# TomClabault/RayTracerCPP

Hardware: NVIDIA B200
Metric: Mrays/s (primary+shadow) (higher is better)
Workload: dtype f32

## Files before the change

### raytracercpp_b200/csrc/kernels.cuh

```cuda
#pragma once

#include <cuda_runtime.h>
#include "rt_device.h"

namespace rtb {

constexpr int kPatch = 8;
constexpr int kPrimaryThreads = 128;
constexpr int kQueueThreads = 128;
constexpr int kPrimaryFetch = 1;
constexpr int kStepsPerCheck = 4;
constexpr unsigned kParkCtas = 296;
constexpr unsigned kFusedGenerations = 12;
constexpr int kItemPasses = 6;
#ifndef RTB_SHADE_MINB
#define RTB_SHADE_MINB 7
#endif

constexpr int kSubQueues = 32;
struct alignas(128) SubQueue {
    unsigned int n;
    unsigned int next;
    unsigned int pad[30];
};
// ... 52 lines not shown
        f += __shfl_xor_sync(0xffffffffu, f, o);
    }
    if ((threadIdx.x & 31u) == 0) {
        if (v) atomicAdd(vol, v);
        if (t) atomicAdd(tri, t);
        if (f) atomicAdd(fetch, f);
    }
}

struct WorkView {
    const uint32_t* tiles;
    uint32_t tile_begin, tile_end;
    int32_t tiles_x;
    int32_t tile_px;
    int32_t patches_per_side;
    int32_t cull_x0, cull_y0, cull_x1, cull_y1;
};

struct QueueView {
    int32_t* slot_tri;
    float* slot_t;
    float* slot_u;
    float* slot_v;
    uint32_t* hit_slot;
    uint32_t* hit_sorted;
    uint32_t sort_mode, sort_slots;
    float* g_z;
    V3* g_n;
    uint32_t* split_base;
    uint32_t* split_active;
    uint32_t* split_occ;
// ... 9 lines not shown
    uint32_t capacity;
};

RT_DEV bool slot_pixel(const WorkView& wk, const FrameView& fr, uint32_t slot, int& px, int& py)
{
    const uint32_t pps = (uint32_t)wk.patches_per_side;
    const uint32_t per_tile = pps * pps * (uint32_t)(kPatch * kPatch);
    const uint32_t tile = wk.tiles[wk.tile_begin + slot / per_tile];
    const uint32_t in_tile = slot % per_tile;
    const uint32_t patch = in_tile / (uint32_t)(kPatch * kPatch), in_patch = in_tile % (uint32_t)(kPatch * kPatch);
    const int lx = (int)(patch % pps) * kPatch + (int)(in_patch & 7u);
    const int ly = (int)(patch / pps) * kPatch + (int)(in_patch >> 3);
    px = (int)(tile % (uint32_t)wk.tiles_x) * wk.tile_px + lx;
    py = (int)(tile / (uint32_t)wk.tiles_x) * wk.tile_px + ly;
    return lx < wk.tile_px && ly < wk.tile_px && px < fr.rw && py < fr.rh;
}

struct Tuning {
    int32_t primary_refill;
    int32_t shade_refill;
    int32_t tri_batch;
    int32_t packets;
    int32_t packet_rounds;
    int32_t item_rounds;
    int32_t primary_rounds;
    int32_t fused;
    int32_t packet_min, item_min, primary_min;
    int32_t item_passes;
    int32_t cull;
};
// ... 455 lines not shown
    uint32_t traced = 0;
    uint32_t nxt = 0;
    if (lane == 0) nxt = atomicAdd(&cnt->next_patch, 32u * kPrimaryFetch);
    for (;;) {
        const uint32_t first = __shfl_sync(0xffffffffu, nxt, 0);
        if (first >= total) break;
        if (lane == 0) nxt = atomicAdd(&cnt->next_patch, 32u * kPrimaryFetch);
#pragma unroll 1
        for (uint32_t b = 0; b < (uint32_t)kPrimaryFetch; b++) {
            const uint32_t base = first + 32u * b;
            if (base >= total) break;
            const uint32_t slot = base + lane;
            int px = 0, py = 0;
            const bool active = slot < total && slot_pixel(wk, fr, slot, px, py);
            V3 o = v3(0, 0, 0), d = v3(0, 0, 1);
            const bool inside = active && px >= wk.cull_x0 && px <= wk.cull_x1 && py >= wk.cull_y0 && py <= wk.cull_y1;
            if (__ballot_sync(0xffffffffu, inside) == 0u) {
                if (slot < total) {
                    q.slot_tri[slot] = -1;
                    if (active) {
                        if (miss_needs_ray(fr)) primary_ray(fr, px, py, o, d);
                        super[(size_t)py * fr.rw + px] = quantise_argb(shade_miss(sc, fr, d));
                    }
                }
                continue;
            }
            if (active) primary_ray(fr, px, py, o, d);
            traced += (uint32_t)__popc(__ballot_sync(0xffffffffu, active));
            HitRec best;
            bool occ, live = active;
            unsigned rounds = 0;
// ... 1173 lines not shown
            backoff = min(backoff * 2u, 4000u);
            continue;
        }
        const uint32_t base = __shfl_sync(0xffffffffu, nxt, 0);
        if (base >= total) {
            more = false;
            if (lane == 0 && my_packets && tune.primary_rounds > 0) { __threadfence(); atomicAdd(&cnt->ft[0].packets_done, my_packets); }
            continue;
        }
        if (lane == 0) nxt = atomicAdd(&cnt->next_patch, 32u);
        rem = (total - base) / per_round;
        const uint32_t slot = base + lane;
        int px = 0, py = 0;
        const bool active = slot_pixel(wk, fr, slot, px, py);
        V3 o = v3(0, 0, 0), d = v3(0, 0, 1);
        const bool inside = active && px >= wk.cull_x0 && px <= wk.cull_x1 && py >= wk.cull_y0 && py <= wk.cull_y1;
        bool deferred = false;
        if (__ballot_sync(0xffffffffu, inside) == 0u) {
            q.slot_tri[slot] = -1;
            if (active) {
                if (miss_needs_ray(fr)) primary_ray(fr, px, py, o, d);
                super[(size_t)py * fr.rw + px] = quantise_argb(shade_miss(sc, fr, d));
            }
        } else {
            if (active) primary_ray(fr, px, py, o, d);
            traced += (uint32_t)__popc(__ballot_sync(0xffffffffu, active));
            HitRec best;
            bool occ, live = active;
            unsigned rounds = 0;
            const unsigned long long t0 = COUNT ? global_ns() : 0ull;
            const bool finished = packet_trace<false, COUNT>(sc, K, top, live, o, d, INFINITY, o, 0.0f, best, occ, tc, overflow,
// ... 183 lines not shown
```

### raytracercpp_b200/csrc/octree_device.cuh

```cuda
#pragma once

#include "scene_layout.h"

namespace rtb {
namespace devbuild {

constexpr int kExtraLevels = 0;
constexpr int kMaxKeyLevels = 21;
constexpr int kSortRounds = 64;
constexpr int kSortUnit = 32 * kSortRounds;
constexpr int kScanItems = 4;
constexpr int kScanBlock = 1024 * kScanItems;

struct Params {
    int32_t max_depth, leaf_max, leaf_split, total_depth;
    float s3;
};

struct Stats {
    unsigned long long interior, nonempty_children;
    unsigned int max_depth, max_leaf;
    unsigned int root_lo[3], root_hi[3];
    unsigned int top_n;
};
// ... 585 lines not shown

__global__ void __launch_bounds__(256)
k_wb_records(const float4* recs, const uint32_t* src, Cells C, uint32_t n_nodes, float4* wrecs)
{
    const uint32_t node = blockIdx.x * blockDim.x + threadIdx.x;
    if (node >= n_nodes) return;
    const float4* s = recs + 4 * (size_t)src[node];
    float4* q = wrecs + 4 * (size_t)C.rec[node];
    float4 q3 = s[3];
    const uint32_t kids = C.info[node] & 15u;
    if (kids) { q3.z = __uint_as_float(C.block[node]); q3.w = __uint_as_float(kids); }
    q[0] = s[0]; q[1] = s[1]; q[2] = s[2]; q[3] = q3;
}

__global__ void __launch_bounds__(256)
k_ob_transform(float* xyz, size_t n_vertices, M4 t)
{
    for (size_t i = (size_t)blockIdx.x * blockDim.x + threadIdx.x; i < n_vertices; i += (size_t)gridDim.x * blockDim.x) {
        const V3 p = xform_point(t, v3(xyz[3 * i], xyz[3 * i + 1], xyz[3 * i + 2]));
        xyz[3 * i] = p.x; xyz[3 * i + 1] = p.y; xyz[3 * i + 2] = p.z;
    }
}

}
}
```

### raytracercpp_b200/csrc/rtb200.cu

```cuda
#include "../../include/rtb200.h"

#include <cuda_runtime.h>
#include <omp.h>
#include <sched.h>

#include <algorithm>
#include <atomic>
#include <chrono>
#include <cmath>
#include <cstdarg>
#include <cstdio>
#include <cstdlib>
#include <cstring>
#include <map>
#include <string>
#include <tuple>
#include <vector>

#include "kernels.cuh"
#include "scene_layout.h"
#include "octree_device.cuh"
#include "light_cull.cuh"
#include "ssao.cuh"
#include "raster.cuh"
#include "host_common.h"

using namespace rtb;

namespace {

constexpr uint64_t kChunkPixels = 1ull << 28;
constexpr int kMaxChunks = 256;

thread_local std::string g_create_error;
std::atomic<unsigned long long> g_alloc_generation{0};

double now_ms()
{
    return std::chrono::duration<double, std::milli>(std::chrono::steady_clock::now().time_since_epoch()).count();
}

template <typename T>
struct DevBuf {
    T* p = nullptr;
    size_t n = 0;
    cudaError_t ensure(size_t count)
    {
// ... 24 lines not shown

struct TimedLaunch {
    int stage;
    cudaEvent_t a, b;
    const char* label;
};

struct TileList {
    uint32_t* d = nullptr;
    uint32_t count = 0;
    int tiles_x = 0;
    std::vector<uint32_t> host;
    uint32_t* d_split = nullptr;
    std::vector<uint32_t> split_host;
    uint32_t n_traced = 0;
    int32_t split_rect[4] = {0, 0, -1, -1};
    int32_t split_tile_px = 0;
    bool split_valid = false;
    float last_hit_fraction = -1.0f;
};
typedef std::tuple<int, int, int, int, int> TileKey;

}

constexpr int kLanes = 2;
constexpr int kMaxLanes = 6;

struct QueueSet {
    DevBuf<uint32_t> hit_slot, refl_idx, split_base, split_active, split_occ, item_ready, split_pending;
    DevBuf<uint32_t> hit_sorted, sort_keys, sort_bins;
    DevBuf<unsigned long long> split_best, refl_cnt;
// ... 16 lines not shown
    bool count = false, shadow = false;
    bool raster = false;
    cudaEvent_t ev_begin = nullptr, ev_end = nullptr;
    uint64_t primary_rays = 0;
    bool has_key = false;
    int key[5] = {0, 0, 0, 0, 0};
    uint64_t traced_slots = 0;
};

struct DeviceBuild {
    DevBuf<float> xyz9, uv6, centroid, c_nr, c_fr;
    DevBuf<int32_t> mat;
    DevBuf<unsigned long long> keys[2];
    DevBuf<uint32_t> idx[2], hist, sums, counts, c_begin, c_end, c_first, c_info, c_size, c_rec, c_block;
    DevBuf<uint32_t> w_src, w_members;
    DevBuf<devbuild::Stats> stats;
    bool tris_on_device = false;
    std::vector<M4> host_pending;
    void release()
    {
        xyz9.release(); uv6.release(); centroid.release(); c_nr.release(); c_fr.release(); mat.release(); keys[0].release(); keys[1].release();
        idx[0].release(); idx[1].release(); hist.release(); sums.release(); counts.release(); c_begin.release(); c_end.release(); c_first.release();
        c_info.release(); c_size.release(); c_rec.release(); c_block.release(); w_src.release(); w_members.release(); stats.release();
    }
};

struct RtContext {
    int device = 0;
    int sm_count = 0;
    cudaStream_t stream = nullptr;
    cudaStream_t own_stream = nullptr;
    std::string error;

    std::vector<float> xyz9, uv6;
    std::vector<int32_t> mat;
    bool has_uv = false, has_mat = false;
    int32_t max_mat_index = -1, min_mat_index = 0;

// ... 54 lines not shown
    DevBuf<RasterUnit> d_runits;
    DevBuf<unsigned int> d_rcount;
    DevBuf<float4> d_rfrag;
    size_t raster_smem_set = 0;
    bool opt_graph = true;
    bool opt_fan_lanes = true;
    bool capturing = false;
    struct FrameGraph { std::string key; cudaGraphExec_t exec; uint32_t launches; };
    std::vector<FrameGraph> graphs;
    std::vector<std::string> seen_keys;
    size_t raster_units0 = (size_t)1 << 18;
    M4 proj{};
    float proj_fov = 45.0f, proj_aspect = 1.0f;
    bool proj_set = false;
    float root_lo[3] = {0, 0, 0}, root_hi[3] = {0, 0, 0};

    bool opt_light_cull = true;
    DevBuf<uint32_t> d_tri_occ, d_blk_occ, d_rec_parent;
    struct LightMaskInputs { V3 light; float span; uint32_t all_set; uint64_t tree; } mask_in{}, mask_next{};
    uint32_t mask_words = 0, mask_recs = 0;
    bool mask_valid = false;
    uint64_t mask_generation = 0;

    DevBuf<float> b_a, b_b, b_t, b_u, b_v;
    DevBuf<int32_t> b_id;
    DevBuf<uint8_t> b_occ;
};

namespace {

// ... 212 lines not shown
        for (int r = c + 1; r < 4; r++) if (std::fabs(m[r][c]) > std::fabs(m[piv][c])) piv = r;
        if (std::fabs(m[piv][c]) < 1e-300) return false;
        if (piv != c) for (int j = 0; j < 8; j++) std::swap(m[piv][j], m[c][j]);
        const double d = 1.0 / m[c][c];
        for (int j = 0; j < 8; j++) m[c][j] *= d;
        for (int r = 0; r < 4; r++) {
            if (r == c) continue;
            const double f = m[r][c];
            if (f != 0.0) for (int j = 0; j < 8; j++) m[r][j] -= f * m[c][j];
        }
    }
    for (int i = 0; i < 4; i++) for (int j = 0; j < 4; j++) out[4 * i + j] = m[i][4 + j];
    return true;
}

void screen_cull_rect(const RtContext* ctx, const FrameView& fr, WorkView& wk)
{
    wk.cull_x0 = 0; wk.cull_y0 = 0; wk.cull_x1 = fr.rw - 1; wk.cull_y1 = fr.rh - 1;
    if (!ctx->opt_screen_cull) return;
    if (ctx->n_tris == 0 || !(ctx->root_lo[0] <= ctx->root_hi[0])) { wk.cull_x0 = 1; wk.cull_x1 = 0; return; }
    double c2w[16], pinv[16], w2c[16], proj[16];
    for (int i = 0; i < 16; i++) { c2w[i] = (&ctx->cam_to_world.m[0][0])[i]; pinv[i] = (&ctx->proj_inv.m[0][0])[i]; }
    if (!invert4(c2w, w2c) || !invert4(pinv, proj)) return;
    const double w0 = c2w[15];
    if (!(std::fabs(w0) > 1e-12)) return;
    const double centre[3] = {c2w[3] / w0, c2w[7] / w0, c2w[11] / w0};
    const double pos[3] = {ctx->cam_pos.x, ctx->cam_pos.y, ctx->cam_pos.z};
    double scale = 1.0;
    for (int k = 0; k < 3; k++) scale = std::max(scale, std::fabs(centre[k]));
    for (int k = 0; k < 3; k++) if (std::fabs(centre[k] - pos[k]) > 1e-5 * scale) return;
    double xmin = 1e300, xmax = -1e300, ymin = 1e300, ymax = -1e300;
    for (int corner = 0; corner < 8; corner++) {
        const double p[4] = {corner & 1 ? ctx->root_hi[0] : ctx->root_lo[0], corner & 2 ? ctx->root_hi[1] : ctx->root_lo[1],
                             corner & 4 ? ctx->root_hi[2] : ctx->root_lo[2], 1.0};
        double v[4], c[4];
        for (int i = 0; i < 4; i++) v[i] = w2c[4 * i] * p[0] + w2c[4 * i + 1] * p[1] + w2c[4 * i + 2] * p[2] + w2c[4 * i + 3] * p[3];
        if (!(std::fabs(v[3]) > 1e-12)) return;
        for (int i = 0; i < 3; i++) v[i] /= v[3];
        v[3] = 1.0;
        for (int i = 0; i < 4; i++) c[i] = proj[4 * i] * v[0] + proj[4 * i + 1] * v[1] + proj[4 * i + 2] * v[2] + proj[4 * i + 3] * v[3];
        if (!(c[3] > 1e-3 * (1.0 + std::fabs(v[2])))) return;
        const double nx = c[0] / c[3], ny = c[1] / c[3];
        if (!std::isfinite(nx) || !std::isfinite(ny)) return;
        xmin = std::min(xmin, nx); xmax = std::max(xmax, nx); ymin = std::min(ymin, ny); ymax = std::max(ymax, ny);
    }
    for (int k = 0; k < 5; k++) {
        const double nx = k == 4 ? 0.0 : (k & 1 ? 1.0 : -1.0), ny = k == 4 ? 0.0 : (k & 2 ? 1.0 : -1.0);
        double v[4];
        for (int i = 0; i < 4; i++) v[i] = pinv[4 * i] * nx + pinv[4 * i + 1] * ny - pinv[4 * i + 2] + pinv[4 * i + 3];
        if (!(std::fabs(v[3]) > 1e-12)) return;
        for (int i = 0; i < 3; i++) v[i] /= v[3];
        for (const double along : {1.0, 7.5}) {
            const double q[4] = {v[0] * along, v[1] * along, v[2] * along, 1.0};
            double c[4];
            for (int i = 0; i < 4; i++) c[i] = proj[4 * i] * q[0] + proj[4 * i + 1] * q[1] + proj[4 * i + 2] * q[2] + proj[4 * i + 3] * q[3];
            if (!(c[3] > 0.0) || !(std::fabs(c[0] / c[3] - nx) < 1e-4) || !(std::fabs(c[1] / c[3] - ny) < 1e-4)) return;
        }
    }
    const double px0 = (xmin + 1.0) * 0.5 * fr.rw, px1 = (xmax + 1.0) * 0.5 * fr.rw;
    const double py0 = (ymin + 1.0) * 0.5 * fr.rh, py1 = (ymax + 1.0) * 0.5 * fr.rh;
    const double lim = 1e9;
    wk.cull_x0 = (int32_t)std::max(-lim, std::floor(px0) - 2.0); wk.cull_x1 = (int32_t)std::min(lim, std::ceil(px1) + 2.0);
    wk.cull_y0 = (int32_t)std::max(-lim, std::floor(py0) - 2.0); wk.cull_y1 = (int32_t)std::min(lim, std::ceil(py1) + 2.0);
}

int get_tile_list(RtContext* ctx, const RtSettings* s, int tile_size, int tile_mod, int tile_rem, TileList** out)
{
    const TileKey key(s->image_width, s->image_height, tile_size, tile_mod, tile_rem);
    auto it = ctx->tile_lists.find(key);
    if (it == ctx->tile_lists.end()) {
        if (ctx->tile_lists.size() > 64) {
            RT_CUDA(ctx, cudaStreamSynchronize(ctx->stream));
            for (auto& kv : ctx->tile_lists) { cudaFree(kv.second.d); cudaFree(kv.second.d_split); }
            ctx->tile_lists.clear();
        }
        TileList tl;
        if (tile_rem >= 0) tl.host = owned_tiles(s, tile_size, tile_mod, tile_rem, &tl.tiles_x);
        else {
// ... 72 lines not shown
}

int scan_counts(RtContext* ctx, uint32_t* data, size_t count, uint32_t* total)
{
    using namespace devbuild;
    DeviceBuild& D = ctx->db;
    const cudaStream_t st = ctx->stream;
    const uint32_t blocks = (uint32_t)((count + kScanBlock - 1) / kScanBlock);
    RT_CUDA(ctx, D.sums.ensure(std::max<uint32_t>(blocks, 1)));
    k_scan_sums<<<blocks, 1024, 0, st>>>(data, count, D.sums.p);
    k_scan_top<<<1, 1024, 0, st>>>(D.sums.p, blocks, total);
    k_scan_apply<<<blocks, 1024, 0, st>>>(data, count, D.sums.p);
    return RT_OK;
}

int build_wide_tree(RtContext* ctx, uint64_t n_records)
{
    using namespace devbuild;
    DeviceBuild& D = ctx->db;
    const cudaStream_t st = ctx->stream;
    const size_t cap = (size_t)n_records;
    RT_CUDA(ctx, D.w_src.ensure(cap)); RT_CUDA(ctx, D.c_first.ensure(cap)); RT_CUDA(ctx, D.c_info.ensure(cap)); RT_CUDA(ctx, D.c_size.ensure(cap));
    RT_CUDA(ctx, D.c_rec.ensure(cap)); RT_CUDA(ctx, D.c_block.ensure(cap)); RT_CUDA(ctx, D.stats.ensure(1));
    Cells C;
    memset(&C, 0, sizeof(C));
    C.first_child = D.c_first.p; C.info = D.c_info.p; C.size = D.c_size.p; C.rec = D.c_rec.p; C.block = D.c_block.p;
    {
        const uint32_t zero = 0u, root_block = 2u;
        RT_CUDA(ctx, cudaMemcpyAsync(D.w_src.p, &zero, 4, cudaMemcpyHostToDevice, st));
        RT_CUDA(ctx, cudaMemcpyAsync(C.rec, &zero, 4, cudaMemcpyHostToDevice, st));
// ... 6 lines not shown
    for (;;) {
        const uint32_t lf = level_first.back(), lc = level_count.back();
        RT_CUDA(ctx, D.counts.ensure(lc));
        RT_CUDA(ctx, D.w_members.ensure(8 * (size_t)lc));
        k_wb_collapse<<<(lc + 255) / 256, 256, 0, st>>>(recs, D.w_src.p, lf, lc, C.info, D.counts.p, D.w_members.p);
        if (int r = scan_counts(ctx, D.counts.p, lc, d_total)) return r;
        uint32_t total = 0;
        RT_CUDA(ctx, cudaMemcpyAsync(&total, d_total, 4, cudaMemcpyDeviceToHost, st));
        RT_CUDA(ctx, cudaStreamSynchronize(st));
        if (total == 0) break;
        if ((size_t)lf + lc + total > cap) return fail(ctx, RT_ERR_STATE, "wide tree: more nodes than child records");
        k_wb_children<<<(lc + 255) / 256, 256, 0, st>>>(C, D.w_src.p, lf, lc, D.counts.p, D.w_members.p, lf + lc);
        level_first.push_back(lf + lc); level_count.push_back(total);
    }
    const uint32_t n_nodes = level_first.back() + level_count.back();
    for (int l = (int)level_first.size() - 1; l >= 0; l--)
        k_wb_size<<<(level_count[l] + 255) / 256, 256, 0, st>>>(C, level_first[l], level_count[l]);
    uint32_t root_size = 0;
    RT_CUDA(ctx, cudaMemcpyAsync(&root_size, C.size, 4, cudaMemcpyDeviceToHost, st));
    RT_CUDA(ctx, cudaStreamSynchronize(st));
    const uint64_t n_wide = 2ull + root_size;
    ctx->n_wrecs = n_wide;
    RT_CUDA(ctx, ctx->d_wrecs.ensure(4 * n_wide));
    RT_CUDA(ctx, cudaMemsetAsync(ctx->d_wrecs.p, 0, 4 * n_wide * sizeof(float4), st));
    Params P;
    memset(&P, 0, sizeof(P));
    for (size_t l = 0; l < level_first.size(); l++)
        k_ob_place<<<(level_count[l] + 255) / 256, 256, 0, st>>>(C, level_first[l], level_count[l], P);
    k_wb_records<<<(n_nodes + 255) / 256, 256, 0, st>>>(recs, D.w_src.p, C, n_nodes, (float4*)ctx->d_wrecs.p);
    k_ob_top_table<<<1, 32, 0, st>>>((float4*)ctx->d_wrecs.p, (float4*)ctx->d_top.p, D.stats.p);
// ... 138 lines not shown
    const bool packets_wide = P.leaf_split > 0;
    if (!packets_wide) k_ob_top_table<<<1, 32, 0, st>>>((float4*)ctx->d_recs.p, (float4*)ctx->d_top.p, D.stats.p);
    Stats hs;
    F4 root_rec[2];
    RT_CUDA(ctx, cudaMemcpyAsync(&hs, D.stats.p, sizeof(hs), cudaMemcpyDeviceToHost, st));
    RT_CUDA(ctx, cudaMemcpyAsync(root_rec, ctx->d_recs.p, sizeof(root_rec), cudaMemcpyDeviceToHost, st));
    RT_CUDA(ctx, cudaStreamSynchronize(st));
    RT_CUDA(ctx, cudaGetLastError());
    ctx->top_n = (int)hs.top_n;
    if (packets_wide) if (int r = build_wide_tree(ctx, n_records)) return r;
    const double t2 = now_ms();

    ctx->n_tris = n32;
    ctx->root_lo[0] = root_rec[0].x; ctx->root_lo[1] = root_rec[0].z; ctx->root_lo[2] = root_rec[1].x;
    ctx->root_hi[0] = root_rec[0].y; ctx->root_hi[1] = root_rec[0].w; ctx->root_hi[2] = root_rec[1].y;
    RtBvhInfo& bi = ctx->info;
    bi.triangles = n;
    bi.interior = hs.interior;
    bi.nodes = 1 + 8 * hs.interior;
    bi.leaves = bi.nodes - bi.interior;
    bi.empty_leaves = 8 * hs.interior - hs.nonempty_children;
    bi.max_depth_reached = hs.max_depth; bi.max_leaf_size = hs.max_leaf;
    bi.child_records = n_records;
    bi.device_bytes = (4 * n_records + 3 * n + 2 * n) * sizeof(F4) + n * sizeof(int32_t);
    bi.build_ms = t2 - t1;
    bi.upload_ms = t1 - t0;
    ctx->bvh_valid = true;
    if (getenv("RTB200_TRACE"))
        fprintf(stderr, "[rtb200] device octree: %u cells on %zu levels, %llu records, upload %.1f ms, build %.1f ms\n", n_cells, level_first.size(),
                (unsigned long long)n_records, t1 - t0, t2 - t1);
// ... 191 lines not shown
    ctx->bvh_valid = false;
    ctx->db.tris_on_device = false;
    ctx->db.host_pending.clear();
    return RT_OK;
}

int rt_build_bvh(RtContext* ctx, int max_depth, int leaf_max_obj_count)
{
    if (!ctx) return RT_ERR_INVALID;
    if (int r = bind(ctx)) return r;
    if (max_depth < 0 || max_depth > RT_MAX_TREE_DEPTH) return fail(ctx, RT_ERR_INVALID, "max_depth %d outside [0,%d]", max_depth, RT_MAX_TREE_DEPTH);
    if (leaf_max_obj_count < 0) return fail(ctx, RT_ERR_INVALID, "leaf_max_obj_count %d", leaf_max_obj_count);
    const size_t n = ctx->xyz9.size() / 9;
    ctx->bvh_valid = false;
    ctx->wide_tree = false;
    ctx->tree_serial++;
    if (ctx->opt_device_build && n > 0) return build_bvh_device(ctx, max_depth, leaf_max_obj_count);
    apply_pending_host_transforms(ctx);
    double t0 = now_ms();
    FlatScene flat;
    build_flat_scene(ctx->xyz9.data(), ctx->has_uv ? ctx->uv6.data() : nullptr, ctx->has_mat ? ctx->mat.data() : nullptr, n,
                     max_depth, leaf_max_obj_count, ctx->opt_leaf_split, flat);
    double t1 = now_ms();
    if (flat.n_records >= (1ull << 28)) return fail(ctx, RT_ERR_INVALID, "scene needs %llu child records (limit 2^28)", (unsigned long long)flat.n_records);
    RT_CUDA(ctx, cudaStreamSynchronize(ctx->stream));
    RT_CUDA(ctx, ctx->d_recs.ensure(flat.recs.size()));
    RT_CUDA(ctx, ctx->d_tris.ensure(flat.tris.size()));
    RT_CUDA(ctx, ctx->d_shade.ensure(flat.shade.size()));
    RT_CUDA(ctx, ctx->d_orig.ensure(flat.orig.size()));
    RT_CUDA(ctx, ctx->d_leaf_of.ensure(flat.orig.size()));
// ... 9 lines not shown
        RT_CUDA(ctx, cudaMemcpyAsync(ctx->d_shade.p, flat.shade.data(), flat.shade.size() * sizeof(F4), cudaMemcpyHostToDevice, ctx->stream));
        RT_CUDA(ctx, cudaMemcpyAsync(ctx->d_orig.p, flat.orig.data(), flat.orig.size() * sizeof(int32_t), cudaMemcpyHostToDevice, ctx->stream));
        RT_CUDA(ctx, cudaMemcpyAsync(ctx->d_leaf_of.p, leaf_of.data(), leaf_of.size() * sizeof(int32_t), cudaMemcpyHostToDevice, ctx->stream));
    }
    RT_CUDA(ctx, cudaStreamSynchronize(ctx->stream));
    double t2 = now_ms();
    if (n && ctx->opt_leaf_split > 0)
        if (int r = build_wide_tree(ctx, flat.n_records)) return r;
    const double wide_ms = now_ms() - t2;
    ctx->n_tris = (uint32_t)n;
    {
        const F4 *q0 = &flat.recs[0], *q1 = &flat.recs[1];
        ctx->root_lo[0] = q0->x; ctx->root_lo[1] = q0->z; ctx->root_lo[2] = q1->x;
        ctx->root_hi[0] = q0->y; ctx->root_hi[1] = q0->w; ctx->root_hi[2] = q1->y;
    }
    RtBvhInfo& bi = ctx->info;
    bi.triangles = n;
    bi.nodes = flat.nodes; bi.leaves = flat.leaves; bi.empty_leaves = flat.empty_leaves; bi.interior = flat.interior;
    bi.max_depth_reached = flat.max_depth_reached; bi.max_leaf_size = flat.max_leaf_size;
    bi.child_records = flat.n_records;
    bi.device_bytes = (flat.recs.size() + flat.tris.size() + flat.shade.size()) * sizeof(F4) + flat.orig.size() * sizeof(int32_t);
    bi.build_ms = t1 - t0 + wide_ms;
    bi.upload_ms = t2 - t1;
    ctx->bvh_valid = true;
    return RT_OK;
}

int rt_bvh_info(const RtContext* ctx, RtBvhInfo* out)
{
    if (!ctx || !out) return RT_ERR_INVALID;
// ... 121 lines not shown
    if (!(aspect > 0.0f) || !(zfar > znear)) return fail(ctx, RT_ERR_INVALID, "projection: aspect %g, znear %g, zfar %g", aspect, znear, zfar);
    ctx->proj = perspective_matrix(fov, aspect, znear, zfar);
    ctx->proj_fov = fov;
    ctx->proj_aspect = aspect;
    ctx->proj_set = true;
    return RT_OK;
}

int rt_set_light(RtContext* ctx, const float position[3])
{
    if (!ctx || !position) return RT_ERR_INVALID;
    ctx->light = v3(position[0], position[1], position[2]);
    return RT_OK;
}

int rt_tile_count(const RtSettings* s, int tile_size, int tile_mod, int tile_rem)
{
    if (!s || tile_size <= 0 || tile_mod <= 0 || tile_rem < 0 || tile_rem >= tile_mod) return RT_ERR_INVALID;
    return (int)owned_tiles(s, tile_size, tile_mod, tile_rem, nullptr).size();
}

int rt_render_device_begin(RtContext* ctx, const RtSettings* s, uint32_t* d_argb_out, int tile_size, int tile_mod, int tile_rem)
{
    if (!ctx) return RT_ERR_INVALID;
    if (ctx->pending.active) return fail(ctx, RT_ERR_STATE, "rt_render_device_begin: the previous frame has not been ended (rt_render_device_end)");
    if (int r = bind(ctx)) return r;
    if (int r = validate_settings(ctx, s)) return r;
    if (int r = validate_scene_for_render(ctx, s)) return r;
    if (int r = check_tile_args(ctx, tile_size, tile_mod, tile_rem)) return r;
    if (!d_argb_out) return fail(ctx, RT_ERR_INVALID, "d_argb_out is NULL");
// ... 10 lines not shown
    const FrameView fr = frame_view(ctx, s);
    const SceneView sc = scene_view(ctx);
    const SceneView scp = packet_view(ctx);
    const bool resolve = fr.factor > 1;
    const bool reflect = ctx->any_reflective && s->shading_method == RT_SHADING;
    if (reflect) if (int r = ensure_stack(ctx, s)) return r;

    TileList* tl = nullptr;
    if (int r = get_tile_list(ctx, s, tile_size, tile_mod, tile_rem, &tl)) return r;
    const std::vector<uint32_t>& owned = tl->host;
    const int tiles_x = tl->tiles_x;
    WorkView wk = {};
    wk.tiles_x = tiles_x;
    wk.tile_px = tile_size * fr.factor;
    wk.patches_per_side = (wk.tile_px + kPatch - 1) / kPatch;
    screen_cull_rect(ctx, fr, wk);
    const bool has_shapes = !ctx->shapes.empty();
    if (has_shapes) { wk.cull_x0 = 0; wk.cull_y0 = 0; wk.cull_x1 = fr.rw - 1; wk.cull_y1 = fr.rh - 1; }
    const bool classify = ctx->opt_screen_cull && ctx->tune.packets && tl->count > 0 && !has_shapes && !raster;
    if (classify) {
        const int32_t rect[4] = {wk.cull_x0, wk.cull_y0, wk.cull_x1, wk.cull_y1};
        if (!tl->split_valid || memcmp(rect, tl->split_rect, sizeof(rect)) != 0 || tl->split_tile_px != wk.tile_px) {
            std::vector<uint32_t> in, out;
            for (uint32_t tile : owned) {
                const int x0 = (int)(tile % (uint32_t)tiles_x) * wk.tile_px, y0 = (int)(tile / (uint32_t)tiles_x) * wk.tile_px;
                const bool hit = !(x0 + wk.tile_px - 1 < rect[0] || x0 > rect[2] || y0 + wk.tile_px - 1 < rect[1] || y0 > rect[3]);
                (hit ? in : out).push_back(tile);
            }
            tl->n_traced = (uint32_t)in.size();
            tl->split_host = in;
            tl->split_host.insert(tl->split_host.end(), out.begin(), out.end());
            if (!tl->d_split) RT_CUDA(ctx, cudaMalloc((void**)&tl->d_split, tl->count * sizeof(uint32_t)));
            RT_CUDA(ctx, cudaStreamSynchronize(ctx->stream));
            RT_CUDA(ctx, cudaMemcpy(tl->d_split, tl->split_host.data(), tl->count * sizeof(uint32_t), cudaMemcpyHostToDevice));
            memcpy(tl->split_rect, rect, sizeof(rect));
            tl->split_tile_px = wk.tile_px;
            tl->split_valid = true;
        }
    }
    const uint32_t n_traced = raster ? 0u : (classify ? tl->n_traced : tl->count);
    const std::vector<uint32_t> tiles(classify ? tl->split_host.begin() : owned.begin(), (classify ? tl->split_host.begin() : owned.begin()) + n_traced);
    const uint64_t px_per_tile = (uint64_t)wk.patches_per_side * wk.patches_per_side * kPatch * kPatch;
    uint32_t tiles_per_chunk = (uint32_t)std::max<uint64_t>(1, ctx->opt_chunk_pixels / px_per_tile);
    if ((tiles.size() + tiles_per_chunk - 1) / tiles_per_chunk > (size_t)kMaxChunks)
        tiles_per_chunk = (uint32_t)((tiles.size() + kMaxChunks - 1) / kMaxChunks);
    const int n_lanes = (ctx->opt_lanes > 1 && tune_packets_hint(ctx)) ? (int)std::min<size_t>((size_t)ctx->opt_lanes, std::max<size_t>(tiles.size(), 1)) : 1;
    if (n_lanes > 1 && tiles.size() <= (size_t)tiles_per_chunk * (n_lanes - 1)) tiles_per_chunk = (uint32_t)((tiles.size() + n_lanes - 1) / n_lanes);
    std::vector<uint32_t> bounds;
    for (size_t b = 0; b < tiles.size(); b += tiles_per_chunk) bounds.push_back((uint32_t)b);
    bounds.push_back((uint32_t)tiles.size());
// ... 101 lines not shown
    bool replay = false, capture = false;
    size_t graph_at = 0;
    std::string key;
    if (graph_ok) {
        auto put = [&](const void* ptr, size_t n) { key.append((const char*)ptr, n); };
        auto put64 = [&](unsigned long long v) { put(&v, sizeof(v)); };
        put(&sc, sizeof(sc)); put(&scp, sizeof(scp)); put(&fr, sizeof(fr)); put(&wk, sizeof(wk)); put(qv, sizeof(QueueView) * (size_t)n_lanes); put(&tune, sizeof(tune));
        put(&light_map, sizeof(light_map));
        if (!bounds.empty()) put(bounds.data(), bounds.size() * sizeof(uint32_t));
        put64((unsigned long long)tile_size); put64((unsigned long long)tile_mod); put64((unsigned long long)tile_rem); put64((unsigned long long)n_lanes);
        put64(n_chunks); put64(classify); put64(n_traced); put64(tl->count); put64((unsigned long long)(uintptr_t)tl->d); put64((unsigned long long)(uintptr_t)tl->d_split);
        put64(sort_hits); put64((unsigned long long)ctx->opt_shadow_sort); put64(tail); put64(psplit); put64(reflect); put64(ssao); put64(resolve); put64(count); put64(has_shapes);
        put64(ctx->opt_top_table); put64((unsigned long long)(uintptr_t)d_argb_out); put64((unsigned long long)(uintptr_t)super);
        put64((unsigned long long)(uintptr_t)ctx->d_counters.p); put64((unsigned long long)(uintptr_t)pd.host_cnt); put64(g_alloc_generation.load());
        put64((unsigned long long)(uintptr_t)main_stream); put64((unsigned long long)split_cap); put64((unsigned long long)item_cap); put64(px_per_tile);
        put64((unsigned long long)ctx->stack_limit_set); put64(ctx->opt_fan_lanes); put64(ctx->mask_generation);
        if (ssao) { put(&ctx->proj, sizeof(ctx->proj)); put(&ctx->proj_fov, sizeof(float)); put(&ctx->proj_aspect, sizeof(float)); }
        for (size_t i = 0; i < ctx->graphs.size() && !replay; i++)
            if (ctx->graphs[i].key == key) { replay = true; graph_at = i; }
        if (!replay) {
            for (const std::string& k : ctx->seen_keys) capture |= (k == key);
            if (!capture) {
                if (ctx->seen_keys.size() >= 4) ctx->seen_keys.erase(ctx->seen_keys.begin());
                ctx->seen_keys.push_back(key);
            }
        }
    }
    cudaEvent_t ev_begin = next_event(ctx), ev_end = next_event(ctx);
    RT_CUDA(ctx, cudaEventRecord(ev_begin, st));
    if (rebuild_masks) if (int r = build_light_masks(ctx, st)) return r;
    auto enqueue = [&]() -> int {
// ... 637 lines not shown
```

Before: 22820.

## Replace screen-space cull rectangle with per-block coverage bitmap from upper tree boxes

Replaces the single screen rectangle (the projected root box) with a bitmap of 8x4 pixel blocks. The bitmap is built on the host by projecting up to 4096 boxes from an upper level of the wide tree, each padded by a conservative error margin. Primary rays in uncovered blocks, and whole tiles with no covered blocks, skip traversal and are shaded as misses. The cost is extra host work and a device-to-host box copy at build time, a bitmap upload when the camera changes, and one bitmap load per ray.

```diff
diff --git a/raytracercpp_b200/csrc/kernels.cuh b/raytracercpp_b200/csrc/kernels.cuh
--- a/raytracercpp_b200/csrc/kernels.cuh
+++ b/raytracercpp_b200/csrc/kernels.cuh
@@ -90,7 +90,8 @@
     int32_t tiles_x;
     int32_t tile_px;
     int32_t patches_per_side;
-    int32_t cull_x0, cull_y0, cull_x1, cull_y1;
+    const uint32_t* cover;
+    int32_t cover_words;
 };
 
 struct QueueView {
@@ -130,6 +131,13 @@
     px = (int)(tile % (uint32_t)wk.tiles_x) * wk.tile_px + lx;
     py = (int)(tile / (uint32_t)wk.tiles_x) * wk.tile_px + ly;
     return lx < wk.tile_px && ly < wk.tile_px && px < fr.rw && py < fr.rh;
+}
+
+RT_DEV bool covered(const WorkView& wk, int px, int py)
+{
+    if (wk.cover == nullptr) return true;
+    const uint32_t w = __ldg(wk.cover + ((uint32_t)py >> 2) * (uint32_t)wk.cover_words + ((uint32_t)px >> 8));
+    return ((w >> (((uint32_t)px >> 3) & 31u)) & 1u) != 0u;
 }
 
 struct Tuning {
@@ -615,7 +623,7 @@
             int px = 0, py = 0;
             const bool active = slot < total && slot_pixel(wk, fr, slot, px, py);
             V3 o = v3(0, 0, 0), d = v3(0, 0, 1);
-            const bool inside = active && px >= wk.cull_x0 && px <= wk.cull_x1 && py >= wk.cull_y0 && py <= wk.cull_y1;
+            const bool inside = active && covered(wk, px, py);
             if (__ballot_sync(0xffffffffu, inside) == 0u) {
                 if (slot < total) {
                     q.slot_tri[slot] = -1;
@@ -1819,7 +1827,7 @@
         int px = 0, py = 0;
         const bool active = slot_pixel(wk, fr, slot, px, py);
         V3 o = v3(0, 0, 0), d = v3(0, 0, 1);
-        const bool inside = active && px >= wk.cull_x0 && px <= wk.cull_x1 && py >= wk.cull_y0 && py <= wk.cull_y1;
+        const bool inside = active && covered(wk, px, py);
         bool deferred = false;
         if (__ballot_sync(0xffffffffu, inside) == 0u) {
             q.slot_tri[slot] = -1;
diff --git a/raytracercpp_b200/csrc/octree_device.cuh b/raytracercpp_b200/csrc/octree_device.cuh
--- a/raytracercpp_b200/csrc/octree_device.cuh
+++ b/raytracercpp_b200/csrc/octree_device.cuh
@@ -623,6 +623,18 @@
 }
 
 __global__ void __launch_bounds__(256)
+k_wb_boxes(const float4* recs, const uint32_t* src, const uint32_t* info, uint32_t n, uint32_t first_kept, float* boxes)
+{
+    const uint32_t node = blockIdx.x * blockDim.x + threadIdx.x;
+    if (node >= n) return;
+    const float4 q0 = recs[4 * (size_t)src[node]], q1 = recs[4 * (size_t)src[node] + 1];
+    const bool keep = node >= first_kept || (info[node] & 15u) == 0u;
+    float* b = boxes + 6 * (size_t)node;
+    b[0] = keep ? q0.x : INFINITY; b[1] = keep ? q0.z : INFINITY; b[2] = keep ? q1.x : INFINITY;
+    b[3] = keep ? q0.y : -INFINITY; b[4] = keep ? q0.w : -INFINITY; b[5] = keep ? q1.y : -INFINITY;
+}
+
+__global__ void __launch_bounds__(256)
 k_ob_transform(float* xyz, size_t n_vertices, M4 t)
 {
     for (size_t i = (size_t)blockIdx.x * blockDim.x + threadIdx.x; i < n_vertices; i += (size_t)gridDim.x * blockDim.x) {
diff --git a/raytracercpp_b200/csrc/rtb200.cu b/raytracercpp_b200/csrc/rtb200.cu
--- a/raytracercpp_b200/csrc/rtb200.cu
+++ b/raytracercpp_b200/csrc/rtb200.cu
@@ -31,6 +31,7 @@
 
 constexpr uint64_t kChunkPixels = 1ull << 28;
 constexpr int kMaxChunks = 256;
+constexpr uint32_t kCoverBoxes = 4096;
 
 thread_local std::string g_create_error;
 std::atomic<unsigned long long> g_alloc_generation{0};
@@ -85,7 +86,7 @@
     uint32_t* d_split = nullptr;
     std::vector<uint32_t> split_host;
     uint32_t n_traced = 0;
-    int32_t split_rect[4] = {0, 0, -1, -1};
+    uint64_t split_cover = 0;
     int32_t split_tile_px = 0;
     bool split_valid = false;
     float last_hit_fraction = -1.0f;
@@ -132,6 +133,7 @@
     DevBuf<unsigned long long> keys[2];
     DevBuf<uint32_t> idx[2], hist, sums, counts, c_begin, c_end, c_first, c_info, c_size, c_rec, c_block;
     DevBuf<uint32_t> w_src, w_members;
+    DevBuf<float> w_boxes;
     DevBuf<devbuild::Stats> stats;
     bool tris_on_device = false;
     std::vector<M4> host_pending;
@@ -139,7 +141,7 @@
     {
         xyz9.release(); uv6.release(); centroid.release(); c_nr.release(); c_fr.release(); mat.release(); keys[0].release(); keys[1].release();
         idx[0].release(); idx[1].release(); hist.release(); sums.release(); counts.release(); c_begin.release(); c_end.release(); c_first.release();
-        c_info.release(); c_size.release(); c_rec.release(); c_block.release(); w_src.release(); w_members.release(); stats.release();
+        c_info.release(); c_size.release(); c_rec.release(); c_block.release(); w_src.release(); w_members.release(); w_boxes.release(); stats.release();
     }
 };
 
@@ -224,6 +226,14 @@
     float proj_fov = 45.0f, proj_aspect = 1.0f;
     bool proj_set = false;
     float root_lo[3] = {0, 0, 0}, root_hi[3] = {0, 0, 0};
+    std::vector<float> cover_boxes;
+    struct CoverInputs { M4 proj_inv, cam_to_world; V3 cam_pos; int32_t rw, rh; uint64_t tree; } cover_in{};
+    bool cover_valid = false;
+    bool cover_bound = false;
+    int32_t cover_words = 0;
+    std::vector<uint32_t> h_cover;
+    DevBuf<uint32_t> d_cover;
+    uint64_t cover_generation = 0;
 
     bool opt_light_cull = true;
     DevBuf<uint32_t> d_tri_occ, d_blk_occ, d_rec_parent;
@@ -466,54 +476,188 @@
     return true;
 }
 
-void screen_cull_rect(const RtContext* ctx, const FrameView& fr, WorkView& wk)
-{
-    wk.cull_x0 = 0; wk.cull_y0 = 0; wk.cull_x1 = fr.rw - 1; wk.cull_y1 = fr.rh - 1;
-    if (!ctx->opt_screen_cull) return;
-    if (ctx->n_tris == 0 || !(ctx->root_lo[0] <= ctx->root_hi[0])) { wk.cull_x0 = 1; wk.cull_x1 = 0; return; }
+bool screen_coverage(const M4& cam_to_world, const M4& proj_inv, V3 cam_pos, int rw, int rh, const float* boxes, size_t n_boxes,
+                     double margin_scale, std::vector<uint32_t>& bits, int32_t& words_per_row)
+{
+    const int bw = (rw + 7) / 8, bh = (rh + 3) / 4;
+    words_per_row = (bw + 31) / 32;
+    bits.assign((size_t)words_per_row * (size_t)bh, 0u);
+    auto set_blocks = [&](int bx0, int by0, int bx1, int by1) {
+        for (int by = by0; by <= by1; by++) {
+            uint32_t* row = bits.data() + (size_t)by * words_per_row;
+            for (int w = bx0 >> 5; w <= bx1 >> 5; w++) {
+                const int lo = std::max(bx0 - 32 * w, 0), hi = std::min(bx1 - 32 * w, 31);
+                row[w] |= (hi == 31 ? 0xffffffffu : ((1u << (hi + 1)) - 1u)) & ~((1u << lo) - 1u);
+            }
+        }
+    };
+    if (n_boxes == 0) return true;
     double c2w[16], pinv[16], w2c[16], proj[16];
-    for (int i = 0; i < 16; i++) { c2w[i] = (&ctx->cam_to_world.m[0][0])[i]; pinv[i] = (&ctx->proj_inv.m[0][0])[i]; }
-    if (!invert4(c2w, w2c) || !invert4(pinv, proj)) return;
+    for (int i = 0; i < 16; i++) { c2w[i] = (&cam_to_world.m[0][0])[i]; pinv[i] = (&proj_inv.m[0][0])[i]; }
+    if (!invert4(c2w, w2c) || !invert4(pinv, proj)) return false;
     const double w0 = c2w[15];
-    if (!(std::fabs(w0) > 1e-12)) return;
+    if (!(std::fabs(w0) > 1e-12)) return false;
     const double centre[3] = {c2w[3] / w0, c2w[7] / w0, c2w[11] / w0};
-    const double pos[3] = {ctx->cam_pos.x, ctx->cam_pos.y, ctx->cam_pos.z};
-    double scale = 1.0;
+    const double pos[3] = {cam_pos.x, cam_pos.y, cam_pos.z};
+    double scale = 1.0, dc = 0.0;
     for (int k = 0; k < 3; k++) scale = std::max(scale, std::fabs(centre[k]));
-    for (int k = 0; k < 3; k++) if (std::fabs(centre[k] - pos[k]) > 1e-5 * scale) return;
-    double xmin = 1e300, xmax = -1e300, ymin = 1e300, ymax = -1e300;
-    for (int corner = 0; corner < 8; corner++) {
-        const double p[4] = {corner & 1 ? ctx->root_hi[0] : ctx->root_lo[0], corner & 2 ? ctx->root_hi[1] : ctx->root_lo[1],
-                             corner & 4 ? ctx->root_hi[2] : ctx->root_lo[2], 1.0};
-        double v[4], c[4];
-        for (int i = 0; i < 4; i++) v[i] = w2c[4 * i] * p[0] + w2c[4 * i + 1] * p[1] + w2c[4 * i + 2] * p[2] + w2c[4 * i + 3] * p[3];
-        if (!(std::fabs(v[3]) > 1e-12)) return;
-        for (int i = 0; i < 3; i++) v[i] /= v[3];
-        v[3] = 1.0;
-        for (int i = 0; i < 4; i++) c[i] = proj[4 * i] * v[0] + proj[4 * i + 1] * v[1] + proj[4 * i + 2] * v[2] + proj[4 * i + 3] * v[3];
-        if (!(c[3] > 1e-3 * (1.0 + std::fabs(v[2])))) return;
-        const double nx = c[0] / c[3], ny = c[1] / c[3];
-        if (!std::isfinite(nx) || !std::isfinite(ny)) return;
-        xmin = std::min(xmin, nx); xmax = std::max(xmax, nx); ymin = std::min(ymin, ny); ymax = std::max(ymax, ny);
-    }
+    for (int k = 0; k < 3; k++) {
+        if (!(std::fabs(centre[k] - pos[k]) <= 1e-5 * scale)) return false;
+        dc += (centre[k] - pos[k]) * (centre[k] - pos[k]);
+    }
+    dc = std::sqrt(dc);
     for (int k = 0; k < 5; k++) {
         const double nx = k == 4 ? 0.0 : (k & 1 ? 1.0 : -1.0), ny = k == 4 ? 0.0 : (k & 2 ? 1.0 : -1.0);
         double v[4];
         for (int i = 0; i < 4; i++) v[i] = pinv[4 * i] * nx + pinv[4 * i + 1] * ny - pinv[4 * i + 2] + pinv[4 * i + 3];
-        if (!(std::fabs(v[3]) > 1e-12)) return;
+        if (!(std::fabs(v[3]) > 1e-12)) return false;
         for (int i = 0; i < 3; i++) v[i] /= v[3];
         for (const double along : {1.0, 7.5}) {
             const double q[4] = {v[0] * along, v[1] * along, v[2] * along, 1.0};
             double c[4];
             for (int i = 0; i < 4; i++) c[i] = proj[4 * i] * q[0] + proj[4 * i + 1] * q[1] + proj[4 * i + 2] * q[2] + proj[4 * i + 3] * q[3];
-            if (!(c[3] > 0.0) || !(std::fabs(c[0] / c[3] - nx) < 1e-4) || !(std::fabs(c[1] / c[3] - ny) < 1e-4)) return;
-        }
-    }
-    const double px0 = (xmin + 1.0) * 0.5 * fr.rw, px1 = (xmax + 1.0) * 0.5 * fr.rw;
-    const double py0 = (ymin + 1.0) * 0.5 * fr.rh, py1 = (ymax + 1.0) * 0.5 * fr.rh;
-    const double lim = 1e9;
-    wk.cull_x0 = (int32_t)std::max(-lim, std::floor(px0) - 2.0); wk.cull_x1 = (int32_t)std::min(lim, std::ceil(px1) + 2.0);
-    wk.cull_y0 = (int32_t)std::max(-lim, std::floor(py0) - 2.0); wk.cull_y1 = (int32_t)std::min(lim, std::ceil(py1) + 2.0);
+            if (!(c[3] > 0.0) || !(std::fabs(c[0] / c[3] - nx) < 1e-4) || !(std::fabs(c[1] / c[3] - ny) < 1e-4)) return false;
+        }
+    }
+    const double eps = 0x1p-24;
+    double VS[3] = {0, 0, 0}, WS[3] = {0, 0, 0}, ws_c[4][3], wmin = 1e300, w2min = 1e300, wsign = 0.0, w2sign = 0.0;
+    for (int k = 0; k < 4; k++) {
+        const double h[4] = {k & 1 ? 1.0 : -1.0, k & 2 ? 1.0 : -1.0, -1.0, 1.0};
+        double vh[4], wh[4];
+        for (int i = 0; i < 4; i++) vh[i] = pinv[4 * i] * h[0] + pinv[4 * i + 1] * h[1] + pinv[4 * i + 2] * h[2] + pinv[4 * i + 3] * h[3];
+        if (k == 0) wsign = vh[3] < 0.0 ? -1.0 : 1.0;
+        if (!(vh[3] * wsign > 0.0)) return false;
+        wmin = std::min(wmin, std::fabs(vh[3]));
+        const double vs[4] = {vh[0] / vh[3], vh[1] / vh[3], vh[2] / vh[3], 1.0};
+        for (int i = 0; i < 4; i++) wh[i] = c2w[4 * i] * vs[0] + c2w[4 * i + 1] * vs[1] + c2w[4 * i + 2] * vs[2] + c2w[4 * i + 3];
+        if (k == 0) w2sign = wh[3] < 0.0 ? -1.0 : 1.0;
+        if (!(wh[3] * w2sign > 0.0)) return false;
+        w2min = std::min(w2min, std::fabs(wh[3]));
+        for (int i = 0; i < 3; i++) {
+            ws_c[k][i] = wh[i] / wh[3];
+            VS[i] = std::max(VS[i], std::fabs(vs[i]));
+            WS[i] = std::max(WS[i], std::fabs(ws_c[k][i]));
+        }
+    }
+    double e1[4], ev[3], e2[4], e3n = 0.0;
+    for (int i = 0; i < 4; i++)
+        e1[i] = 6.0 * eps * (std::fabs(pinv[4 * i]) + std::fabs(pinv[4 * i + 1]) + std::fabs(pinv[4 * i + 2]) + std::fabs(pinv[4 * i + 3]));
+    if (!(wmin > 2.0 * e1[3])) return false;
+    for (int i = 0; i < 3; i++) ev[i] = (e1[i] + VS[i] * e1[3]) / (wmin - e1[3]) + 2.0 * eps * VS[i];
+    for (int i = 0; i < 4; i++) {
+        double s2 = std::fabs(c2w[4 * i + 3]), p2 = 0.0;
+        for (int j = 0; j < 3; j++) { s2 += std::fabs(c2w[4 * i + j]) * VS[j]; p2 += std::fabs(c2w[4 * i + j]) * ev[j]; }
+        e2[i] = 4.0 * eps * s2 + p2;
+    }
+    if (!(w2min > 2.0 * e2[3])) return false;
+    for (int i = 0; i < 3; i++) {
+        const double ew = (e2[i] + WS[i] * e2[3]) / (w2min - e2[3]) + 2.0 * eps * WS[i];
+        const double e3 = ew + eps * (WS[i] + std::fabs(pos[i]));
+        e3n += e3 * e3;
+    }
+    e3n = std::sqrt(e3n);
+    double u[3], v[3], n[3];
+    for (int i = 0; i < 3; i++) { u[i] = ws_c[1][i] - ws_c[0][i]; v[i] = ws_c[2][i] - ws_c[0][i]; }
+    n[0] = u[1] * v[2] - u[2] * v[1]; n[1] = u[2] * v[0] - u[0] * v[2]; n[2] = u[0] * v[1] - u[1] * v[0];
+    const double nn = std::sqrt(n[0] * n[0] + n[1] * n[1] + n[2] * n[2]);
+    const double lmin = std::fabs(n[0] * (ws_c[0][0] - pos[0]) + n[1] * (ws_c[0][1] - pos[1]) + n[2] * (ws_c[0][2] - pos[2])) / nn;
+    if (!(lmin > 4.0 * e3n)) return false;
+    const double e_dir = 2.0 * e3n / lmin + 5.0 * eps;
+    const double kTriRel = 0x1p-14;
+    const double pos_max = std::max(std::fabs(pos[0]), std::max(std::fabs(pos[1]), std::fabs(pos[2])));
+    const double ndc_slack = 1e-9;
+    for (size_t b = 0; b < n_boxes; b++) {
+        const float* bx = boxes + 6 * b;
+        bool finite = true, empty = false;
+        double lo[3], hi[3], bmax = 0.0;
+        for (int k = 0; k < 3; k++) {
+            lo[k] = bx[k]; hi[k] = bx[3 + k];
+            finite &= std::isfinite(lo[k]) && std::isfinite(hi[k]);
+            empty |= lo[k] > hi[k];
+            bmax = std::max(bmax, std::max(std::fabs(lo[k]), std::fabs(hi[k])));
+        }
+        if (empty) continue;
+        if (!finite) { set_blocks(0, 0, bw - 1, bh - 1); return true; }
+        double sfar = 0.0;
+        for (int c = 0; c < 8; c++) {
+            double d2 = 0.0;
+            for (int k = 0; k < 3; k++) { const double x = ((c >> k) & 1 ? hi[k] : lo[k]) - pos[k]; d2 += x * x; }
+            sfar = std::max(sfar, std::sqrt(d2));
+        }
+        const double e_tri = kTriRel * (pos_max + bmax + sfar);
+        const double reach = (sfar + e_tri) * (1.0 + 5.0 * eps);
+        const double r = margin_scale * (e_tri + reach * e_dir + dc * (2.0 + reach / lmin));
+        double xmin = 1e300, xmax = -1e300, ymin = 1e300, ymax = -1e300;
+        bool whole = false;
+        for (int c = 0; c < 8 && !whole; c++) {
+            const double p[4] = {(c & 1 ? hi[0] + r : lo[0] - r), (c & 2 ? hi[1] + r : lo[1] - r), (c & 4 ? hi[2] + r : lo[2] - r), 1.0};
+            double vv[4], cc[4];
+            for (int i = 0; i < 4; i++) vv[i] = w2c[4 * i] * p[0] + w2c[4 * i + 1] * p[1] + w2c[4 * i + 2] * p[2] + w2c[4 * i + 3] * p[3];
+            if (!(std::fabs(vv[3]) > 1e-12)) { whole = true; break; }
+            for (int i = 0; i < 3; i++) vv[i] /= vv[3];
+            vv[3] = 1.0;
+            for (int i = 0; i < 4; i++) cc[i] = proj[4 * i] * vv[0] + proj[4 * i + 1] * vv[1] + proj[4 * i + 2] * vv[2] + proj[4 * i + 3] * vv[3];
+            if (!(cc[3] > 1e-3 * (1.0 + std::fabs(vv[2])))) { whole = true; break; }
+            const double nx = cc[0] / cc[3], ny = cc[1] / cc[3];
+            if (!std::isfinite(nx) || !std::isfinite(ny)) { whole = true; break; }
+            xmin = std::min(xmin, nx); xmax = std::max(xmax, nx); ymin = std::min(ymin, ny); ymax = std::max(ymax, ny);
+        }
+        if (whole) { set_blocks(0, 0, bw - 1, bh - 1); return true; }
+        const double lim = 1e9;
+        const double px0 = std::ceil(std::max(-lim, (xmin - ndc_slack + 1.0) * 0.5 * rw - 0.5)), px1 = std::floor(std::min(lim, (xmax + ndc_slack + 1.0) * 0.5 * rw - 0.5));
+        const double py0 = std::ceil(std::max(-lim, (ymin - ndc_slack + 1.0) * 0.5 * rh - 0.5)), py1 = std::floor(std::min(lim, (ymax + ndc_slack + 1.0) * 0.5 * rh - 0.5));
+        const int x0 = (int)std::max(0.0, px0), x1 = (int)std::min((double)rw - 1, px1);
+        const int y0 = (int)std::max(0.0, py0), y1 = (int)std::min((double)rh - 1, py1);
+        if (x0 > x1 || y0 > y1) continue;
+        set_blocks(x0 >> 3, y0 >> 2, x1 >> 3, y1 >> 2);
+    }
+    return true;
+}
+
+bool cover_any(const std::vector<uint32_t>& bits, int32_t words_per_row, int x0, int y0, int x1, int y1)
+{
+    const int bx0 = x0 >> 3, bx1 = x1 >> 3;
+    for (int by = y0 >> 2; by <= y1 >> 2; by++) {
+        const uint32_t* row = bits.data() + (size_t)by * words_per_row;
+        for (int w = bx0 >> 5; w <= bx1 >> 5; w++) {
+            const int lo = std::max(bx0 - 32 * w, 0), hi = std::min(bx1 - 32 * w, 31);
+            if (row[w] & (hi == 31 ? 0xffffffffu : ((1u << (hi + 1)) - 1u)) & ~((1u << lo) - 1u)) return true;
+        }
+    }
+    return false;
+}
+
+int update_cover(RtContext* ctx, const FrameView& fr)
+{
+    RtContext::CoverInputs in;
+    memset(&in, 0, sizeof(in));
+    in.proj_inv = ctx->proj_inv; in.cam_to_world = ctx->cam_to_world; in.cam_pos = ctx->cam_pos;
+    in.rw = fr.rw; in.rh = fr.rh; in.tree = ctx->tree_serial;
+    if (ctx->cover_valid && memcmp(&in, &ctx->cover_in, sizeof(in)) == 0) return RT_OK;
+    ctx->cover_valid = false;
+    const double t0 = now_ms();
+    ctx->cover_bound = screen_coverage(ctx->cam_to_world, ctx->proj_inv, ctx->cam_pos, fr.rw, fr.rh, ctx->cover_boxes.data(),
+                                       ctx->cover_boxes.size() / 6, 1.0, ctx->h_cover, ctx->cover_words);
+    const double t1 = now_ms();
+    double t2 = t1;
+    if (ctx->cover_bound) {
+        RT_CUDA(ctx, cudaStreamSynchronize(ctx->stream));
+        t2 = now_ms();
+        RT_CUDA(ctx, ctx->d_cover.ensure(ctx->h_cover.size()));
+        RT_CUDA(ctx, cudaMemcpyAsync(ctx->d_cover.p, ctx->h_cover.data(), ctx->h_cover.size() * sizeof(uint32_t), cudaMemcpyHostToDevice, ctx->stream));
+    }
+    static const bool trace = getenv("RTB200_TRACE") != nullptr;
+    if (trace) {
+        size_t set = 0;
+        for (uint32_t w : ctx->h_cover) set += (size_t)__builtin_popcount(w);
+        const size_t blocks = (size_t)((fr.rw + 7) / 8) * (size_t)((fr.rh + 3) / 4);
+        fprintf(stderr, "[rtb200] screen coverage: %zu boxes, bound %d, %.4f of the blocks covered, build %.3f ms, upload %.3f ms\n",
+                ctx->cover_boxes.size() / 6, (int)ctx->cover_bound, ctx->cover_bound ? (double)set / (double)blocks : 1.0, t1 - t0, now_ms() - t2);
+    }
+    ctx->cover_in = in;
+    ctx->cover_valid = true;
+    ctx->cover_generation++;
+    return RT_OK;
 }
 
 int get_tile_list(RtContext* ctx, const RtSettings* s, int tile_size, int tile_mod, int tile_rem, TileList** out)
@@ -616,6 +760,11 @@
     return RT_OK;
 }
 
+void root_cover_box(RtContext* ctx)
+{
+    ctx->cover_boxes.assign({ctx->root_lo[0], ctx->root_lo[1], ctx->root_lo[2], ctx->root_hi[0], ctx->root_hi[1], ctx->root_hi[2]});
+}
+
 int build_wide_tree(RtContext* ctx, uint64_t n_records)
 {
     using namespace devbuild;
@@ -652,6 +801,16 @@
         level_first.push_back(lf + lc); level_count.push_back(total);
     }
     const uint32_t n_nodes = level_first.back() + level_count.back();
+    {
+        size_t lv = 0;
+        while (lv + 1 < level_first.size() && level_count[lv + 1] <= kCoverBoxes) lv++;
+        const uint32_t n_box = level_first[lv] + level_count[lv];
+        RT_CUDA(ctx, D.w_boxes.ensure(6 * (size_t)n_box));
+        k_wb_boxes<<<(n_box + 255) / 256, 256, 0, st>>>(recs, D.w_src.p, C.info, n_box, level_first[lv], D.w_boxes.p);
+        ctx->cover_boxes.resize(6 * (size_t)n_box);
+        RT_CUDA(ctx, cudaMemcpyAsync(ctx->cover_boxes.data(), D.w_boxes.p, 6 * (size_t)n_box * sizeof(float), cudaMemcpyDeviceToHost, st));
+        RT_CUDA(ctx, cudaStreamSynchronize(st));
+    }
     for (int l = (int)level_first.size() - 1; l >= 0; l--)
         k_wb_size<<<(level_count[l] + 255) / 256, 256, 0, st>>>(C, level_first[l], level_count[l]);
     uint32_t root_size = 0;
@@ -820,6 +979,7 @@
     ctx->n_tris = n32;
     ctx->root_lo[0] = root_rec[0].x; ctx->root_lo[1] = root_rec[0].z; ctx->root_lo[2] = root_rec[1].x;
     ctx->root_hi[0] = root_rec[0].y; ctx->root_hi[1] = root_rec[0].w; ctx->root_hi[2] = root_rec[1].y;
+    if (!ctx->wide_tree) root_cover_box(ctx);
     RtBvhInfo& bi = ctx->info;
     bi.triangles = n;
     bi.interior = hs.interior;
@@ -1041,6 +1201,7 @@
     const size_t n = ctx->xyz9.size() / 9;
     ctx->bvh_valid = false;
     ctx->wide_tree = false;
+    ctx->cover_boxes.clear();
     ctx->tree_serial++;
     if (ctx->opt_device_build && n > 0) return build_bvh_device(ctx, max_depth, leaf_max_obj_count);
     apply_pending_host_transforms(ctx);
@@ -1080,6 +1241,7 @@
         ctx->root_lo[0] = q0->x; ctx->root_lo[1] = q0->z; ctx->root_lo[2] = q1->x;
         ctx->root_hi[0] = q0->y; ctx->root_hi[1] = q0->w; ctx->root_hi[2] = q1->y;
     }
+    if (!ctx->wide_tree && n) root_cover_box(ctx);
     RtBvhInfo& bi = ctx->info;
     bi.triangles = n;
     bi.nodes = flat.nodes; bi.leaves = flat.leaves; bi.empty_leaves = flat.empty_leaves; bi.interior = flat.interior;
@@ -1231,6 +1393,21 @@
     return RT_OK;
 }
 
+int rt_screen_coverage(const float proj_inv[16], const float cam_to_world[16], const float position[3], int rw, int rh,
+                       const float* boxes, size_t n_boxes, double margin_scale, uint32_t* bits, size_t n_words)
+{
+    if (!proj_inv || !cam_to_world || !position || rw <= 0 || rh <= 0 || (n_boxes && !boxes) || !bits) return RT_ERR_INVALID;
+    M4 pinv, c2w;
+    memcpy(pinv.m, proj_inv, 64);
+    memcpy(c2w.m, cam_to_world, 64);
+    std::vector<uint32_t> out;
+    int32_t words = 0;
+    const bool bound = screen_coverage(c2w, pinv, v3(position[0], position[1], position[2]), rw, rh, boxes, n_boxes, margin_scale, out, words);
+    if (out.size() > n_words) return RT_ERR_INVALID;
+    std::copy(out.begin(), out.end(), bits);
+    return bound ? 1 : 0;
+}
+
 int rt_tile_count(const RtSettings* s, int tile_size, int tile_mod, int tile_rem)
 {
     if (!s || tile_size <= 0 || tile_mod <= 0 || tile_rem < 0 || tile_rem >= tile_mod) return RT_ERR_INVALID;
@@ -1271,17 +1448,19 @@
     wk.tiles_x = tiles_x;
     wk.tile_px = tile_size * fr.factor;
     wk.patches_per_side = (wk.tile_px + kPatch - 1) / kPatch;
-    screen_cull_rect(ctx, fr, wk);
     const bool has_shapes = !ctx->shapes.empty();
-    if (has_shapes) { wk.cull_x0 = 0; wk.cull_y0 = 0; wk.cull_x1 = fr.rw - 1; wk.cull_y1 = fr.rh - 1; }
-    const bool classify = ctx->opt_screen_cull && ctx->tune.packets && tl->count > 0 && !has_shapes && !raster;
+    const bool cull = ctx->opt_screen_cull && ctx->tune.packets && !has_shapes && !raster;
+    if (cull) if (int r = update_cover(ctx, fr)) return r;
+    wk.cover = (cull && ctx->cover_bound) ? ctx->d_cover.p : nullptr;
+    wk.cover_words = wk.cover ? ctx->cover_words : 0;
+    const bool classify = wk.cover != nullptr && tl->count > 0;
     if (classify) {
-        const int32_t rect[4] = {wk.cull_x0, wk.cull_y0, wk.cull_x1, wk.cull_y1};
-        if (!tl->split_valid || memcmp(rect, tl->split_rect, sizeof(rect)) != 0 || tl->split_tile_px != wk.tile_px) {
+        if (!tl->split_valid || tl->split_cover != ctx->cover_generation || tl->split_tile_px != wk.tile_px) {
             std::vector<uint32_t> in, out;
             for (uint32_t tile : owned) {
                 const int x0 = (int)(tile % (uint32_t)tiles_x) * wk.tile_px, y0 = (int)(tile / (uint32_t)tiles_x) * wk.tile_px;
-                const bool hit = !(x0 + wk.tile_px - 1 < rect[0] || x0 > rect[2] || y0 + wk.tile_px - 1 < rect[1] || y0 > rect[3]);
+                const int x1 = std::min(x0 + wk.tile_px, fr.rw) - 1, y1 = std::min(y0 + wk.tile_px, fr.rh) - 1;
+                const bool hit = cover_any(ctx->h_cover, ctx->cover_words, x0, y0, x1, y1);
                 (hit ? in : out).push_back(tile);
             }
             tl->n_traced = (uint32_t)in.size();
@@ -1290,7 +1469,7 @@
             if (!tl->d_split) RT_CUDA(ctx, cudaMalloc((void**)&tl->d_split, tl->count * sizeof(uint32_t)));
             RT_CUDA(ctx, cudaStreamSynchronize(ctx->stream));
             RT_CUDA(ctx, cudaMemcpy(tl->d_split, tl->split_host.data(), tl->count * sizeof(uint32_t), cudaMemcpyHostToDevice));
-            memcpy(tl->split_rect, rect, sizeof(rect));
+            tl->split_cover = ctx->cover_generation;
             tl->split_tile_px = wk.tile_px;
             tl->split_valid = true;
         }
@@ -1422,7 +1601,7 @@
         put64(ctx->opt_top_table); put64((unsigned long long)(uintptr_t)d_argb_out); put64((unsigned long long)(uintptr_t)super);
         put64((unsigned long long)(uintptr_t)ctx->d_counters.p); put64((unsigned long long)(uintptr_t)pd.host_cnt); put64(g_alloc_generation.load());
         put64((unsigned long long)(uintptr_t)main_stream); put64((unsigned long long)split_cap); put64((unsigned long long)item_cap); put64(px_per_tile);
-        put64((unsigned long long)ctx->stack_limit_set); put64(ctx->opt_fan_lanes); put64(ctx->mask_generation);
+        put64((unsigned long long)ctx->stack_limit_set); put64(ctx->opt_fan_lanes); put64(ctx->mask_generation); put64(ctx->cover_generation);
         if (ssao) { put(&ctx->proj, sizeof(ctx->proj)); put(&ctx->proj_fov, sizeof(float)); put(&ctx->proj_aspect, sizeof(float)); }
         for (size_t i = 0; i < ctx->graphs.size() && !replay; i++)
             if (ctx->graphs[i].key == key) { replay = true; graph_at = i; }
```

After: 25070, median of 6. +9.9%, better.
